# opencb/hpg-variant

Measured on AMD Instinct MI355X. Metric: variants/s chi2 assoc, higher is better.
Workload: dtype u8

## Files before the change

### hpg-variant_amd/csrc/hpgv_capi.hip

```cpp
#include "hpgv_internal.h"
#include <cstdlib>

extern "C" {

const char *hpgv_version(void) { return "hpgv-mi355x 0.1 (gfx950)"; }

int hpgv_device_count(void) {
    int n = 0;
    if (hipGetDeviceCount(&n) != hipSuccess) return -1;
    return n;
}

const char *hpgv_last_error(const hpgv_ctx *ctx) { return ctx ? ctx->err.c_str() : g_create_error.c_str(); }

static void read_environment(hpgv_ctx *ctx) {
    auto num = [](const char *name, long lo, long hi, long *out) { const char *e = getenv(name); if (e && *e) { long v = atol(e); *out = v < lo ? lo : v > hi ? hi : v; } };
    num("HPGV_BATCH_COPY", 0, 1, &ctx->batch_copy);
    num("HPGV_BATCH_FUSED", 0, 1, &ctx->batch_fused);
    num("HPGV_STATS_ALL2", 0, 1, &ctx->stats_all2);
    num("HPGV_ASSOC_ROWS", 0, 1, &ctx->assoc_rows);
    num("HPGV_PINNED_NONCOHERENT", 0, 1, &ctx->pinned_noncoherent);
    num("HPGV_VMM_TRACE", 0, 1, &ctx->vmm_trace);
    num("HPGV_DECODE_TILES", 0, 1, &ctx->decode_tiles);
#ifdef HPGV_ABLATION
// ... 127 lines not shown
        if (s->stream) (void)hipStreamDestroy(s->stream);
        delete s;
    }
    for (int i = 0; i < 4; ++i) if (ctx->ev[i]) (void)hipEventDestroy(ctx->ev[i]);
    delete ctx;
}

#ifdef HPGV_ABLATION
#define HPGV_SHIPPED_ONLY(ok, what)
#else
#define HPGV_SHIPPED_ONLY(ok, what) if (!(ok)) return fail(ctx, HPGV_ERR_UNSUPPORTED, what ": that form is an ablation build's (-DHPGV_ABLATION, tools/build_ablation.py)");
#endif

int hpgv_set_option(hpgv_ctx *ctx, const char *key, long value) {
    if (is_group(ctx) && key && !strcmp(key, "group_self_exchange")) { ctx->group_self_exchange = value ? 1 : 0; return HPGV_OK; }
    if (is_group(ctx) && key && !strcmp(key, "group_fake_ranks")) {
        if (value < 0 || value > 65536) return fail(ctx, HPGV_ERR_INVALID, "group_fake_ranks must be 0 (ranks by distinct device) or the number of members that share rank 0");
        std::lock_guard<std::mutex> lk(ctx->mu);
        if (ctx->grp) return fail(ctx, HPGV_ERR_STATE, "group_fake_ranks must be set before the group's communicator exists (hpgv_group_comm_init, the first group call)");
        ctx->group_fake_ranks = value;
        return HPGV_OK;
    }
    GROUP_ALL(ctx, hpgv_set_option(m_, key, value))
    if (!ctx || !key) return HPGV_ERR_INVALID;
    if (!strcmp(key, "row_align")) {
        if (value < 16 || (value & (value - 1))) return fail(ctx, HPGV_ERR_INVALID, "row_align must be a power of two >= 16");
        if (ctx->assoc.set || ctx->tdt.set || ctx->stats.set)
            return fail(ctx, HPGV_ERR_STATE, "row_align must be set before the cohort");
        ctx->row_align = value;
    } else if (!strcmp(key, "row_pad")) {
        if (value < 0 || value % 16 || value > 65536) return fail(ctx, HPGV_ERR_INVALID, "row_pad must be a multiple of 16 in [0, 65536]");
        if (ctx->assoc.set || ctx->tdt.set || ctx->stats.set)
            return fail(ctx, HPGV_ERR_STATE, "row_pad must be set before the cohort");
        ctx->row_pad = value;
    } else if (!strcmp(key, "variants_per_wave")) {
        if (value < 1 || value > 1024) return fail(ctx, HPGV_ERR_INVALID, "variants_per_wave out of range");
        ctx->vpw = value;
    } else if (!strcmp(key, "nontemporal")) {
        HPGV_SHIPPED_ONLY(value != 0, "nontemporal = 0")
        ctx->nontemporal = value ? 1 : 0;
    } else if (!strcmp(key, "profile")) {
        ctx->profile = value ? 1 : 0;
    } else if (!strcmp(key, "scan_unroll")) {
        if (value != 4 && value != 8 && value != 10 && value != 12 && value != 16)
            return fail(ctx, HPGV_ERR_INVALID, "scan_unroll must be one of 4, 8, 10, 12, 16");
        HPGV_SHIPPED_ONLY(value == 4, "scan_unroll other than 4")
        ctx->scan_unroll = value;
    } else if (!strcmp(key, "pipeline")) {
        HPGV_SHIPPED_ONLY(value != 0, "pipeline = 0")
        ctx->pipeline = value ? 1 : 0;
    } else if (!strcmp(key, "fisher_cut_exp")) {
        if (value < 12 || value > 300) return fail(ctx, HPGV_ERR_INVALID, "fisher_cut_exp must be in [12, 300]");
        ctx->fisher_cut_exp = value;
    } else if (!strcmp(key, "epi_complete")) {
        ctx->epi_complete = value ? 1 : 0;
    } else if (!strcmp(key, "epi_triples_mfma")) {
        ctx->epi_triples_mfma = value ? 1 : 0;
    } else if (!strcmp(key, "epi_pairs_mfma")) {
        ctx->epi_pairs_mfma = value ? 1 : 0;
    } else if (!strcmp(key, "epi_wide")) {
        if (value < 0 || value > 2) return fail(ctx, HPGV_ERR_INVALID, "epi_wide must be 0 (the packed kernels' limits), 1 (the wide kernel where the shape needs it) or 2 (the wide kernel for every listed-combination launch)");
        ctx->epi_wide = value;
    } else if (!strcmp(key, "epi_triples_1pass")) {
        if (value < 0 || value > 2) return fail(ctx, HPGV_ERR_INVALID, "epi_triples_1pass must be 0 (two passes), 1 (the cells nine at a time) or 2 (one pass, one wave per SIMD)");
        HPGV_SHIPPED_ONLY(value != 2, "epi_triples_1pass = 2")
        ctx->epi_triples_1pass = value;
    } else if (!strcmp(key, "scan_lds")) {
        if (value < 0 || value > 160 * 1024) return fail(ctx, HPGV_ERR_INVALID, "scan_lds must be in [0, 163840]");
        ctx->scan_lds = value;
    } else if (!strcmp(key, "batch_copy")) {
        ctx->batch_copy = value ? 1 : 0;
    } else if (!strcmp(key, "inflate_wave")) {
        if (value < 0 || value > 4) return fail(ctx, HPGV_ERR_INVALID, "inflate_wave must be 0 (lane per block), 1 (by the number of blocks), 2 (wave per block), 4 (wave per block, several symbols per round) or 3 (lane per block, symbol tables in LDS)");
        HPGV_SHIPPED_ONLY(value == 1 || value == 4, "inflate_wave other than 1 / 4 (a wave per block, several symbols per round)")
        ctx->inflate_wave = value;
    } else if (!strcmp(key, "tokenizer_tiles")) {
        if (value < 0 || value > 2) return fail(ctx, HPGV_ERR_INVALID, "tokenizer_tiles must be 2 (one sweep), 1 (two sweeps) or 0 (line by line)");
        HPGV_SHIPPED_ONLY(value == 1, "tokenizer_tiles other than 1 (two sweeps)")
        ctx->tokenizer_tiles = value;
    } else if (!strcmp(key, "fisher_width")) {
        if (value != 64 && value != 32 && value != 16 && value != 8) return fail(ctx, HPGV_ERR_INVALID, "fisher_width must be 64, 32, 16 or 8");
        HPGV_SHIPPED_ONLY(value == 16, "fisher_width other than 16")
        ctx->fisher_width = value;
    } else if (!strcmp(key, "batch_fused")) {
        ctx->batch_fused = value ? 1 : 0;
    } else if (!strcmp(key, "pipe_waves")) {
        if (value != 4 && value != 6 && value != 8) return fail(ctx, HPGV_ERR_INVALID, "pipe_waves must be 4, 6 or 8");
        HPGV_SHIPPED_ONLY(value == 4, "pipe_waves other than 4")
        ctx->pipe_waves = value;
    } else if (!strcmp(key, "persistent")) {
        HPGV_SHIPPED_ONLY(value == 0, "persistent = 1")
        ctx->persistent = value ? 1 : 0;
    } else if (!strcmp(key, "part_aligned_loads")) {
        HPGV_SHIPPED_ONLY(value == 0, "part_aligned_loads = 1")
        ctx->part_aligned = value ? 1 : 0;
    } else if (!strcmp(key, "pca_apply_vector")) {
        HPGV_SHIPPED_ONLY(value == 0, "pca_apply_vector = 1")
        ctx->pca_apply_vector = value ? 1 : 0;
    } else if (!strcmp(key, "blocks_per_cu")) {
        if (value < 1 || value > 8) return fail(ctx, HPGV_ERR_INVALID, "blocks_per_cu must be in 1..8");
        ctx->blocks_per_cu = value;
    } else {
        return fail(ctx, HPGV_ERR_INVALID, "unknown option '%s'", key);
    }
    return HPGV_OK;
}


int hpgv_set_cohort(hpgv_ctx *ctx, const uint8_t *condition, int n_samples) {
    HPGV_ABI_TRY
    GROUP_ALL(ctx, hpgv_set_cohort(m_, condition, n_samples))
    if (!ctx) return HPGV_ERR_INVALID;
    if (!condition || n_samples < 0) return fail(ctx, HPGV_ERR_INVALID, "bad cohort arguments");
    DeviceGuard g(ctx->device);
    int nA = 0, nU = 0;
    for (int j = 0; j < n_samples; ++j) {
        if (condition[j] == HPGV_COND_AFFECTED) nA++;
        else if (condition[j] == HPGV_COND_UNAFFECTED) nU++;
    }
    size_t segA = round_up((size_t)nA, 16), segU = round_up((size_t)nU, 16);
    size_t pitch = round_up(segA + segU, (size_t)ctx->row_align) + (size_t)ctx->row_pad;
    if (pitch == 0) pitch = (size_t)ctx->row_align;
    if (!pitch_supported(pitch)) return fail(ctx, HPGV_ERR_UNSUPPORTED, "cohort of %d samples exceeds the row-length limit", n_samples);
    Layout &L = ctx->assoc;
    ctx->n_perms = ctx->perm_rows = 0;
    ctx->n_covar = 0;
    ctx->has_pheno = false; ctx->lin_y.clear(); ctx->lin_cov.clear();
    L.n_samples = n_samples;
    L.pitch = pitch;
    L.col_of_pos.assign(pitch, -1);
    size_t a = 0, u = segA;
    for (int j = 0; j < n_samples; ++j) {
        if (condition[j] == HPGV_COND_AFFECTED) L.col_of_pos[a++] = j;
        else if (condition[j] == HPGV_COND_UNAFFECTED) L.col_of_pos[u++] = j;
    }
    ctx->nA = nA; ctx->nU = nU; ctx->chunksA = (int)(segA / 16);
    {
        std::vector<uint8_t> cond(round_up((size_t)n_samples, 16) + 16, (uint8_t)HPGV_COND_OTHER);
        for (int j = 0; j < n_samples; ++j) cond[(size_t)j] = condition[j] == HPGV_COND_AFFECTED ? 1 : condition[j] == HPGV_COND_UNAFFECTED ? 0 : 2;
        HIPCHK(ctx, ctx->d_cond.reserve(cond.size()));
        HIPCHK(ctx, hipMemcpy(ctx->d_cond.p, cond.data(), cond.size(), hipMemcpyHostToDevice));
    }
    return upload_layout(ctx, L);
    HPGV_ABI_CATCH(ctx)
}

int hpgv_assoc_layout(const hpgv_ctx *ctx, int *n_affected, int *n_unaffected, size_t *pitch) {
    ctx = first_member(ctx);
    if (!ctx) return HPGV_ERR_INVALID;
    if (!ctx->assoc.set) return fail(ctx, HPGV_ERR_STATE, "hpgv_set_cohort has not been called");
    if (n_affected) *n_affected = ctx->nA;
    if (n_unaffected) *n_unaffected = ctx->nU;
    if (pitch) *pitch = ctx->assoc.pitch;
    return HPGV_OK;
}

int hpgv_set_logfact(hpgv_ctx *ctx, const double *table, size_t n) {
    GROUP_ALL(ctx, hpgv_set_logfact(m_, table, n))
    if (!ctx) return HPGV_ERR_INVALID;
    if (!table || n == 0) return fail(ctx, HPGV_ERR_INVALID, "empty log-factorial table");
    DeviceGuard g(ctx->device);
    ctx->n_lf = 0;
    if (ctx->cap_lf < n) {
        if (ctx->d_lf_base) { (void)hipFree(ctx->d_lf_base); ctx->d_lf_base = nullptr; ctx->d_lf = nullptr; ctx->cap_lf = 0; }
        HIPCHK(ctx, hipMalloc(&ctx->d_lf_base, (n + 4) * sizeof(double)));
        HIPCHK(ctx, hipMemset(ctx->d_lf_base, 0, (n + 4) * sizeof(double)));
// ... 423 lines not shown
```

### hpg-variant_amd/csrc/hpgv_internal.h

```cpp
#pragma once
#include "../../include/hpgv.h"
#include "hpgv_kernels.h"
#include "hpgv_tdt_stats_kernels.h"
#include "hpgv_epi_kernels.h"

#include <hip/hip_runtime.h>
#include <cctype>

#include <algorithm>
#include <atomic>
#include <cmath>
#include <cstdarg>
#include <cstdio>
#include <cstring>
#include <mutex>
#include <new>
#include <string>
#include <vector>

namespace { thread_local std::string g_create_error; }

struct DevBuf {
    void *p = nullptr;
    size_t cap = 0;
// ... 74 lines not shown

struct TextMeta {
    char *base;
    size_t max_lines;
    TextMeta(const DevBuf &meta, int max_lines_) : base(meta.as<char>()), max_lines((size_t)max_lines_) {}
    static size_t bytes(int max_lines) { return 16 + ((size_t)max_lines + 2) * sizeof(uint64_t) + (size_t)max_lines * 10 * sizeof(uint32_t) + 16; }
    int *n_lines() const { return (int *)base; }
    unsigned long long *line_off() const { return (unsigned long long *)(base + 16); }
    uint32_t *field_off() const { return (uint32_t *)(base + 16 + (max_lines + 2) * sizeof(uint64_t)); }
};

struct Staged {
    const uint8_t *d_raw = nullptr;
    size_t raw_pitch = 0;
    const uint8_t *d_laid = nullptr;
    int which = 0;
    const uint8_t *d_isx = nullptr;
    int n = 0;
    size_t out_stride = 0;
    bool text = false;
};

struct EpiState {
    bool have_data = false, have_folds = false;
    int V = 0, nA = 0, nU = 0, num_folds = 0, W = 0, V_alloc = 0, n_chunks = 0;
    bool wide_only = false;
    int fold_cap = 0;
    int rank_fold_cap = 0;
    uint8_t *d_data = nullptr;
    uint32_t *d_planes = nullptr;
    uint32_t rev_off = 0;
    hpgv_epi_rank_info rank_info{};
    uint32_t *d_marg = nullptr;
    bool complete = false;
    hpgv::EpiChunk *d_chunks = nullptr;
    uint32_t *d_chunk_cls = nullptr;
    hpgv::EpiFold *d_folds = nullptr;
    uint32_t *d_group_w0 = nullptr;
    std::vector<int32_t> group_size;
    DevBuf cand;
    unsigned *d_cand_count = nullptr;
    unsigned cand_cap = 0;
    double *d_thr = nullptr;
    DevBuf tile_base;
};

struct hpgv_ctx {
    std::vector<hpgv_ctx *> members;
    hpgv_ctx *parent = nullptr;
    struct GroupState *grp = nullptr;
    long group_self_exchange = 0;
    long group_fake_ranks = 0;
    std::atomic<unsigned> deal_next{0};
    std::atomic<int> in_flight{0};
    int device = 0;
    mutable std::string err;
    std::mutex mu;
    long row_align = 16;
    long row_pad = 0;
    long vpw = 2;
    long nontemporal = 1;
    long profile = 0;
    std::mutex alias_mu;
    std::vector<std::pair<const char *, const char *>> text_alias;
    struct TextTiles { const char *d_text, *d_base; const void *d_tiles; uint64_t n_tiles; };
    std::vector<TextTiles> text_tiles;
    struct TextHeld { const char *host_text; Slot *slot; const char *d_text; const unsigned long long *d_line_off; int n_lines; };
    std::vector<TextHeld> text_held;
    long part_aligned = 0;
    long pca_apply_vector = 0;
    long scan_unroll = 4;
    long persistent = 0;
    long blocks_per_cu = 8;
    long pipeline = 1;
    long pipe_waves = 4;
    long fisher_cut_exp = 22;
    long epi_complete = 1;
    long epi_pairs_mfma = 1;
    long epi_triples_mfma = 1;
    long epi_wide = 0;
    long epi_triples_1pass = 1;
    long scan_lds = 0;
    long fisher_width = 16;
    long inflate_wave = 1;
    long tokenizer_tiles = 1;
    long batch_copy = 0;
    long batch_fused = 1;
    long batch_lds_max = 65536;
    long stats_all2 = 1;
    long assoc_rows = 1;
    long pinned_noncoherent = 0;
    long vmm_trace = 0;
    long decode_tiles = 1;
#ifdef HPGV_ABLATION
    long stats_rows = 0, stats_bs = 0, stats_debug = 0;
    long fisher_lds = 0;
    long inflate_lds_pad = 0, inflate_wave_wgs = 0, inflate_lane_wgs = 0;
#endif
    int n_cus = 256;
    Layout assoc;
    int nA = 0, nU = 0, chunksA = 0;
    DevBuf d_cond;
    DevBuf d_perm;
    int n_perms = 0, perm_rows = 0;
    DevBuf d_cov;
    int n_covar = 0;
    std::vector<double> lin_y, lin_cov;
    bool has_pheno = false;
    DevBuf d_lin;
    Layout tdt;
    hpgv::TdtPlan tdt_plan;
    DevBuf d_flips;
    int n_flips = 0, flip_rows = 0, flip_pitch = 0;
    int tdt_families = 0;
    DevBuf d_flip_tail;
    Layout stats;
    Layout sgroups;
    std::vector<uint32_t> sg_off;
    std::vector<int> sg_size;
    DevBuf d_sg_chunks;
    DevBuf d_group_of_col;
    bool all_grouped = false;
    Layout mendel;
    int mendel_trios = 0, mendel_pchunks = 0;
    hpgv::MendelLuts mendel_luts{};
    uint8_t *d_mendel_male = nullptr;
    double *d_lf = nullptr;
    double *d_lf_base = nullptr;
    size_t n_lf = 0;
    size_t cap_lf = 0;
    DevBuf d_thr;
    hipEvent_t ev[4] = {nullptr, nullptr, nullptr, nullptr};
    bool have_scan_ev = false, have_stats_ev = false;
    std::vector<Slot *> slots;
    uint32_t *d_sink = nullptr;
    uint32_t *d_crc_tab = nullptr;
    struct TokScratch {
        hipStream_t stream = nullptr;
        DevBuf blocks, line_off, extra;
    };
    std::mutex tok_mu;
    std::vector<TokScratch *> tok_scratch;
    struct GrowRange { char *base = nullptr; size_t reserved = 0, committed = 0; std::vector<hipMemGenericAllocationHandle_t> pieces; std::vector<size_t> sizes; };
    std::vector<GrowRange> grow;
    double filt_min_maf = -1.0, filt_max_missing = -1.0;
    long filt_max_mendel = -1;
    double filt_min_dom = -1.0, filt_min_rec = -1.0;
    std::mutex epi_mu;
    EpiState epi;
};

namespace {

[[maybe_unused]] int fail(const hpgv_ctx *ctx, int code, const char *fmt, ...) {
    char buf[512];
    va_list ap;
    va_start(ap, fmt);
    vsnprintf(buf, sizeof buf, fmt, ap);
    va_end(ap);
    if (ctx) {
        ctx->err = buf;
        if (ctx->parent) {
            std::lock_guard<std::mutex> lk(ctx->parent->mu);
            ctx->parent->err = buf;
        }
    } else g_create_error = buf;
// ... 193 lines not shown
```

### hpg-variant_amd/csrc/hpgv_scan_capi.hip

```cpp
#include "hpgv_internal.h"
#include <type_traits>
#include "hpgv_inherit_kernels.h"

namespace {

unsigned scan_blocks(const hpgv_ctx *ctx, int n_variants) {
    const long waves = ((long)n_variants + ctx->vpw - 1) / ctx->vpw;
    return (unsigned)((waves + 3) / 4);
}

const char *const kAligned16 = "device buffers must be 16-byte aligned";
int scan_checks(hpgv_ctx *ctx, int n_variants, const void *d_gt, const void *d_out, uintptr_t out_mask, const char *align_text, bool *go) {
    *go = false;
    if (n_variants < 0 || (n_variants > 0 && (!d_gt || !d_out))) return fail(ctx, HPGV_ERR_INVALID, "bad scan arguments");
    if (n_variants == 0) return HPGV_OK;
    if (((uintptr_t)d_gt & 15) || ((uintptr_t)d_out & out_mask)) return fail(ctx, HPGV_ERR_INVALID, "%s", align_text);
    *go = true;
    return HPGV_OK;
}

template <typename F>
void launch_nt(const hpgv_ctx *ctx, F &&f) {
    if (ctx->nontemporal) f(std::true_type{}); else f(std::false_type{});
}

}

extern "C" {


static Layout *pick_layout(hpgv_ctx *ctx, int which) {
    switch (which) {
        case HPGV_LAYOUT_ASSOC: return &ctx->assoc;
        case HPGV_LAYOUT_TDT: return &ctx->tdt;
        case HPGV_LAYOUT_STATS: return &ctx->stats;
        case HPGV_LAYOUT_STATS_GROUPS: return &ctx->sgroups;
        case HPGV_LAYOUT_MENDEL: return &ctx->mendel;
        case HPGV_LAYOUT_EPI: return &ctx->assoc;
        default: return nullptr;
    }
}

static void recode_of(const hpgv_ctx *ctx, int which, int *mode, int *p16) {
    *mode = hpgv::RECODE_NONE; *p16 = 0;
    if (which == HPGV_LAYOUT_TDT) { *mode = hpgv::RECODE_TDT; *p16 = ctx->tdt_plan.p16; }
    else if (which == HPGV_LAYOUT_STATS || which == HPGV_LAYOUT_STATS_GROUPS) { *mode = hpgv::RECODE_STATS; }
    else if (which == HPGV_LAYOUT_MENDEL) { *mode = hpgv::RECODE_MENDEL; }
    else if (which == HPGV_LAYOUT_EPI) { *mode = hpgv::RECODE_EPI; }
}

int hpgv_layout_dev(hpgv_ctx *ctx, int which, const uint8_t *d_src, size_t src_pitch, int n_variants,
                    uint8_t *d_dst, void *stream) {
    ctx = first_member(ctx);
    if (!ctx) return HPGV_ERR_INVALID;
    Layout *L = pick_layout(ctx, which);
    if (!L) return fail(ctx, HPGV_ERR_INVALID, "unknown layout %d", which);
    if (!L->set) return fail(ctx, HPGV_ERR_STATE, "layout %d has no cohort yet", which);
    if (n_variants < 0 || (n_variants > 0 && (!d_src || !d_dst))) return fail(ctx, HPGV_ERR_INVALID, "bad layout arguments");
    if (src_pitch < (size_t)L->n_samples) return fail(ctx, HPGV_ERR_INVALID, "src_pitch %zu < n_samples %d", src_pitch, L->n_samples);
    if (n_variants == 0) return HPGV_OK;
    DeviceGuard g(ctx->device);
    const int strict = (which == HPGV_LAYOUT_STATS || which == HPGV_LAYOUT_STATS_GROUPS) ? 0 : 1;
    int mode, p16;
    recode_of(ctx, which, &mode, &p16);
    const long slab = std::max(1L, (1L << 31) / (L->chunks > 0 ? L->chunks : 1));
    for (long off = 0; off < n_variants; off += slab) {
        const int n = (int)std::min(slab, (long)n_variants - off);
        const long total = (long)n * L->chunks;
        hipLaunchKernelGGL(hpgv::k_layout, dim3((unsigned)((total + 255) / 256)), dim3(256), 0, (hipStream_t)stream,
                           d_src + (size_t)off * src_pitch, src_pitch, n, L->pitch, L->chunks, L->d_col_of_pos(), strict, mode, p16,
                           d_dst + (size_t)off * L->pitch);
    }
    HIPCHK(ctx, hipGetLastError());
    return HPGV_OK;
}

static int synth_common(hpgv_ctx *ctx, uint64_t v0, int n_variants, size_t pitch, int chunks,
                        const int32_t *d_col, int mode, int p16, uint8_t *d_dst, hipStream_t st) {
    const long by_threads = (1L << 31) / (chunks > 0 ? chunks : 1);
    const int slab = (int)std::max(1L, std::min((long)(1 << 20), by_threads));
    HIPCHK(ctx, ctx->d_thr.reserve((size_t)(n_variants < slab ? n_variants : slab) * 3 * sizeof(uint32_t)));
    uint32_t *d_thr = ctx->d_thr.as<uint32_t>();
    for (int off = 0; off < n_variants; off += slab) {
        const int n = (n_variants - off) < slab ? (n_variants - off) : slab;
        hipLaunchKernelGGL(hpgv::k_synth_thresholds, dim3((n + 255) / 256), dim3(256), 0, st,
// ... 62 lines not shown
    unsigned blocks = scan_blocks(ctx, n_variants);
    if (ctx->persistent) {
        const unsigned cap = (unsigned)(ctx->n_cus * ctx->blocks_per_cu);
        const unsigned need = (unsigned)(((long)n_variants + 3) / 4);
        blocks = need < cap ? need : cap;
    }
    hipStream_t st = (hipStream_t)stream;
    const uint8_t *gt = d_gt;
    int4 *out = (int4 *)d_counts;
    const int cA = ctx->chunksA, ch = L.chunks;
    const size_t pitch = L.pitch;
#define HPGV_LAUNCH_PIPE(NT, U, W)                                                                \
    hipLaunchKernelGGL((hpgv::k_assoc_scan_pipe<NT, U, W>), dim3(blocks), dim3(256), 0, st, gt, pitch, \
                       n_variants, cA, ch, d_is_x, out, vpw)
#ifndef HPGV_ABLATION
    return launch_profiled(ctx, st, 0, [&] { HPGV_LAUNCH_PIPE(true, 4, 4); });
#else
#define HPGV_LAUNCH_ASSOC(NT, U, S)                                                              \
    hipLaunchKernelGGL((hpgv::k_assoc_scan<NT, U, S>), dim3(blocks), dim3(256), 0, st, gt, pitch, \
                       n_variants, cA, ch, d_is_x, out, vpw)
#define HPGV_DISPATCH_U(NT, S)                                                                   \
    switch (ctx->scan_unroll) {                                                                  \
        case 4: HPGV_LAUNCH_ASSOC(NT, 4, S); break;                                              \
        case 10: HPGV_LAUNCH_ASSOC(NT, 10, S); break;                                            \
        case 12: HPGV_LAUNCH_ASSOC(NT, 12, S); break;                                            \
        case 16: HPGV_LAUNCH_ASSOC(NT, 16, S); break;                                            \
        default: HPGV_LAUNCH_ASSOC(NT, 8, S); break;                                             \
    }
#define HPGV_PIPE_W(NT, U)                                                                       \
    do {                                                                                         \
        if (ctx->pipe_waves == 8) { HPGV_LAUNCH_PIPE(NT, U, 8); }                                \
        else if (ctx->pipe_waves == 6) { HPGV_LAUNCH_PIPE(NT, U, 6); }                           \
        else { HPGV_LAUNCH_PIPE(NT, U, 4); }                                                     \
    } while (0)
    if (ctx->pipeline && !ctx->persistent)
        return launch_profiled(ctx, st, 0, [&] {
            if (ctx->nontemporal) {
                if (ctx->scan_unroll <= 4) HPGV_PIPE_W(true, 4); else HPGV_PIPE_W(true, 5);
            } else {
                if (ctx->scan_unroll <= 4) HPGV_PIPE_W(false, 4); else HPGV_PIPE_W(false, 5);
            }
        });
    return launch_profiled(ctx, st, 0, [&] {
        if (ctx->nontemporal) {
            if (ctx->persistent) { HPGV_DISPATCH_U(true, true) } else { HPGV_DISPATCH_U(true, false) }
        } else {
            if (ctx->persistent) { HPGV_DISPATCH_U(false, true) } else { HPGV_DISPATCH_U(false, false) }
        }
    });
#undef HPGV_DISPATCH_U
#undef HPGV_PIPE_W
#undef HPGV_LAUNCH_ASSOC
#endif
#undef HPGV_LAUNCH_PIPE
}

int hpgv_assoc_chisq_dev(hpgv_ctx *ctx, const int32_t *d_counts, int n_variants, double *d_odds,
                         double *d_chisq, double *d_p, void *stream) {
    ctx = first_member(ctx);
    if (!ctx) return HPGV_ERR_INVALID;
    if (n_variants < 0 || (n_variants > 0 && (!d_counts || !d_odds || !d_chisq || !d_p)))
        return fail(ctx, HPGV_ERR_INVALID, "bad chisq arguments");
    if (n_variants == 0) return HPGV_OK;
    DeviceGuard g(ctx->device);
    hipStream_t st = (hipStream_t)stream;
    return launch_profiled(ctx, st, 1, [&] {
        hipLaunchKernelGGL(hpgv::k_assoc_chisq, dim3((n_variants + 255) / 256), dim3(256), 0, st,
                           (const int4 *)d_counts, n_variants, d_odds, d_chisq, d_p);
    });
}

int hpgv_assoc_fisher_dev(hpgv_ctx *ctx, const int32_t *d_counts, int n_variants, double *d_odds,
                          double *d_p, void *stream) {
    ctx = first_member(ctx);
    if (!ctx) return HPGV_ERR_INVALID;
    if (n_variants < 0 || (n_variants > 0 && (!d_counts || !d_odds || !d_p)))
        return fail(ctx, HPGV_ERR_INVALID, "bad fisher arguments");
    if (const int rc = logfact_check(ctx)) return rc;
    if (n_variants == 0) return HPGV_OK;
    DeviceGuard g(ctx->device);
    hipStream_t st = (hipStream_t)stream;
    const double cut = pow(10.0, -(double)ctx->fisher_cut_exp);
    return launch_profiled(ctx, st, 1, [&] {
        const long per_block = 4 * (64 / ctx->fisher_width);
        const unsigned blocks = (unsigned)(((long)n_variants + per_block - 1) / per_block);
#ifdef HPGV_ABLATION
        const unsigned pad = (unsigned)ctx->fisher_lds;
        if (ctx->fisher_width == 64)
            hipLaunchKernelGGL(hpgv::k_assoc_fisher<64>, dim3(blocks), dim3(256), pad, st, (const int4 *)d_counts, n_variants, ctx->d_lf, d_odds, d_p, cut);
        else if (ctx->fisher_width == 8)
            hipLaunchKernelGGL(hpgv::k_assoc_fisher<8>, dim3(blocks), dim3(256), pad, st, (const int4 *)d_counts, n_variants, ctx->d_lf, d_odds, d_p, cut);
        else if (ctx->fisher_width == 32)
            hipLaunchKernelGGL(hpgv::k_assoc_fisher<32>, dim3(blocks), dim3(256), pad, st, (const int4 *)d_counts, n_variants, ctx->d_lf, d_odds, d_p, cut);
        else
#else
        const unsigned pad = 0u;
#endif
            hipLaunchKernelGGL(hpgv::k_assoc_fisher<16>, dim3(blocks), dim3(256), pad, st, (const int4 *)d_counts, n_variants, ctx->d_lf, d_odds, d_p, cut);
    });
}


int hpgv_tdt_scan_dev(hpgv_ctx *ctx, const uint8_t *d_gt, int n_variants, const uint8_t *d_is_x,
                      int32_t *d_tu, void *stream) {
    ctx = first_member(ctx);
    if (!ctx) return HPGV_ERR_INVALID;
    if (!ctx->tdt.set) return fail(ctx, HPGV_ERR_STATE, "hpgv_set_families has not been called");
    bool go;
    if (const int rc = scan_checks(ctx, n_variants, d_gt, d_tu, 7, "device buffers must be aligned", &go); rc || !go) return rc;
    DeviceGuard g(ctx->device);
    hipStream_t st = (hipStream_t)stream;
    return launch_profiled(ctx, st, 0, [&] {
        ctx->tdt_plan.launch_scan(d_gt, ctx->tdt.pitch, n_variants, d_is_x, (int2 *)d_tu,
                                  (int)ctx->vpw, ctx->nontemporal != 0, st);
    });
}

int hpgv_tdt_stats_dev(hpgv_ctx *ctx, const int32_t *d_tu, int n_variants, double *d_odds,
                       double *d_chisq, double *d_p, void *stream) {
    ctx = first_member(ctx);
    if (!ctx) return HPGV_ERR_INVALID;
    if (n_variants < 0 || (n_variants > 0 && (!d_tu || !d_odds || !d_chisq || !d_p)))
        return fail(ctx, HPGV_ERR_INVALID, "bad tdt stats arguments");
    if (n_variants == 0) return HPGV_OK;
    DeviceGuard g(ctx->device);
    hipStream_t st = (hipStream_t)stream;
    return launch_profiled(ctx, st, 1, [&] {
        hipLaunchKernelGGL(hpgv::k_tdt_stats, dim3((n_variants + 255) / 256), dim3(256), 0, st,
                           (const int2 *)d_tu, n_variants, d_odds, d_chisq, d_p);
    });
}


static int stats_scan(hpgv_ctx *ctx, const Layout &L, const uint8_t *d_gt, int n_variants, uint32_t off, int chunks, size_t lds,
                      int32_t *d_counts8, hipStream_t st) {
    bool go;
    if (const int rc = scan_checks(ctx, n_variants, d_gt, d_counts8, 15, kAligned16, &go); rc || !go) return rc;
    DeviceGuard g(ctx->device);
    const int vpw = (int)ctx->vpw;
    const unsigned blocks = scan_blocks(ctx, n_variants);
    return launch_profiled(ctx, st, 0, [&] {
        launch_nt(ctx, [&](auto NT) {
            constexpr bool nt = decltype(NT)::value;
            if (ctx->pipeline)
                hipLaunchKernelGGL((hpgv::k_stats_scan_hs<nt>), dim3(blocks), dim3(256), nt ? lds : 0, st, d_gt, L.pitch, n_variants, off, chunks, (int4 *)d_counts8, vpw);
            else
                hipLaunchKernelGGL((hpgv::k_stats_scan<nt, kScanUnroll>), dim3(blocks), dim3(256), 0, st, d_gt, L.pitch, n_variants, off, chunks, (int4 *)d_counts8, vpw);
        });
    });
}

int hpgv_stats_scan_dev(hpgv_ctx *ctx, const uint8_t *d_gt, int n_variants, int32_t *d_counts8, void *stream) {
    ctx = first_member(ctx);
    if (!ctx) return HPGV_ERR_INVALID;
    if (!ctx->stats.set) return fail(ctx, HPGV_ERR_STATE, "hpgv_set_stats_cohort has not been called");
    const Layout &L = ctx->stats;
    const size_t scan_lds = ctx->scan_lds > 0 ? (size_t)ctx->scan_lds : (L.pitch >= 6656 ? (size_t)49152 : (size_t)0);
    return stats_scan(ctx, L, d_gt, n_variants, 0u, L.chunks, scan_lds, d_counts8, (hipStream_t)stream);
}

int hpgv_stats_scan_group_dev(hpgv_ctx *ctx, const uint8_t *d_gt, int n_variants, int group, int32_t *d_counts8, void *stream) {
    ctx = first_member(ctx);
    if (!ctx) return HPGV_ERR_INVALID;
    if (!ctx->sgroups.set) return fail(ctx, HPGV_ERR_STATE, "hpgv_set_stats_groups has not been called");
    if (group < 0 || (size_t)group >= ctx->sg_off.size()) return fail(ctx, HPGV_ERR_INVALID, "group %d out of range", group);
    const int chunks = (int)(round_up((size_t)ctx->sg_size[(size_t)group], 16) / 16);
    return stats_scan(ctx, ctx->sgroups, d_gt, n_variants, ctx->sg_off[(size_t)group], chunks, 0, d_counts8, (hipStream_t)stream);
}

int hpgv_stats_hwe_dev(hpgv_ctx *ctx, const int32_t *d_counts8, int n_variants, double *d_chi2,
                       double *d_p, void *stream) {
    ctx = first_member(ctx);
    if (!ctx) return HPGV_ERR_INVALID;
    if (n_variants < 0 || (n_variants > 0 && (!d_counts8 || !d_chi2 || !d_p)))
        return fail(ctx, HPGV_ERR_INVALID, "bad hwe arguments");
    if (n_variants == 0) return HPGV_OK;
    DeviceGuard g(ctx->device);
    hipStream_t st = (hipStream_t)stream;
    return launch_profiled(ctx, st, 1, [&] {
        hipLaunchKernelGGL(hpgv::k_stats_hwe, dim3((n_variants + 255) / 256), dim3(256), 0, st,
                           (const int4 *)d_counts8, n_variants, d_chi2, d_p);
// ... 152 lines not shown
```

Measured before the change: 136.7 million.

## Add packed Fisher kernel that load-balances tail sums across tables in a wave

Adds a new Fisher exact test kernel in which each wave handles four contingency tables. It locates the significant tail ranges with ballot-based window searches, then spreads the tail-term evaluation evenly across all 64 lanes through an LDS work list. It also uses a leaner exp with a cutoff derived from the tail-decay estimate. The aim is to cut lane imbalance when tables differ in tail length, at the cost of more LDS use and a more complex kernel. It becomes the default Fisher path, but chi-square association does not go through it.

```diff
diff --git a/hpg-variant_amd/csrc/hpgv_capi.hip b/hpg-variant_amd/csrc/hpgv_capi.hip
--- a/hpg-variant_amd/csrc/hpgv_capi.hip
+++ b/hpg-variant_amd/csrc/hpgv_capi.hip
@@ -233,6 +233,9 @@
         if (value != 64 && value != 32 && value != 16 && value != 8) return fail(ctx, HPGV_ERR_INVALID, "fisher_width must be 64, 32, 16 or 8");
         HPGV_SHIPPED_ONLY(value == 16, "fisher_width other than 16")
         ctx->fisher_width = value;
+    } else if (!strcmp(key, "fisher_packed")) {
+        HPGV_SHIPPED_ONLY(value != 0, "fisher_packed = 0")
+        ctx->fisher_packed = value ? 1 : 0;
     } else if (!strcmp(key, "batch_fused")) {
         ctx->batch_fused = value ? 1 : 0;
     } else if (!strcmp(key, "pipe_waves")) {
diff --git a/hpg-variant_amd/csrc/hpgv_fisher_kernels.h b/hpg-variant_amd/csrc/hpgv_fisher_kernels.h
--- /dev/null
+++ b/hpg-variant_amd/csrc/hpgv_fisher_kernels.h
@@ -0,0 +1,250 @@
+#pragma once
+#include "hpgv_kernels.h"
+
+namespace hpgv {
+
+constexpr int FISHER_PACK_TABLES = 4;
+constexpr int FISHER_PACK_TAILS = 2 * FISHER_PACK_TABLES;
+constexpr int FISHER_PACK_SLOTS = 64;
+
+struct alignas(16) FisherTail {
+    double konst; int pb8, n ;
+    int r1c, c1c, d0c, pq ;
+    int s16 , q , pad0, pad1;
+};
+
+__device__ __forceinline__ void fisher_wave_sync() {
+    __builtin_amdgcn_fence(__ATOMIC_RELEASE, "wavefront");
+    __builtin_amdgcn_wave_barrier();
+    __builtin_amdgcn_fence(__ATOMIC_ACQUIRE, "wavefront");
+}
+
+__device__ __forceinline__ double fisher_exp_lean(double e, const double *tab , bool keep) {
+    const double t = e * 0x1.71547652b82fep+6 + 0x1.8p+52;
+    const double kf = t - 0x1.8p+52;
+    const int ki = (int)(uint32_t)(uint64_t)__double_as_longlong(t);
+    double r = __builtin_fma(-kf, 0x1.62e42fe000000p-7, e);
+    r = __builtin_fma(-kf, 0x1.f473de6af278fp-36, r);
+    const double tj = tab[ki & 63];
+    double q = __builtin_fma(r, 1.0 / 120.0, 1.0 / 24.0);
+    q = __builtin_fma(r, q, 1.0 / 6.0);
+    q = __builtin_fma(r, q, 0.5);
+    q = __builtin_fma(r * r, q, r);
+    const double y = __builtin_fma(tj, q, tj);
+    return __builtin_ldexp(y, keep ? ki >> 6 : -4000);
+}
+
+
+__device__ __forceinline__ double fisher_get(double v, int lane, int k) { return __shfl(v, (lane & ~15) + k); }
+
+__device__ __forceinline__ void fisher_count2x16(bool p_lo, bool p_hi, int lane, int *left, int *right) {
+    const uint64_t bl = __ballot(p_lo), bh = __ballot(p_hi);
+    const uint32_t l = (((lane & 32) ? (uint32_t)(bl >> 32) : (uint32_t)bl) >> (lane & 16)) & 0xffffu;
+    const uint32_t h = (((lane & 32) ? (uint32_t)(bh >> 32) : (uint32_t)bh) >> (lane & 16)) & 0xffffu;
+    *left = __builtin_popcount(l & 0xffu) + __builtin_popcount(h & 0xffu);
+    *right = __builtin_popcount(l >> 8) + __builtin_popcount(h >> 8);
+}
+
+__device__ __forceinline__ bool fisher_windows_shared(const FisherTab &T, double thr , int mode, int obs, int lane,
+                                                      int *L1, int *R1, int *L2, int *R2) {
+    constexpr int W = 16;
+    const int sl = sub_lane<W>(lane), right = sl >> 3, j = sl & 7;
+    const int g1 = obs <= mode ? obs + 1 : 2 * mode - obs + 1, g2 = obs <= mode ? 2 * mode - obs : obs;
+    int w1 = g1 - W / 2, w2 = g2 - W / 2;
+    w1 = w1 > *R1 - W ? *R1 - W : w1; w1 = w1 < *L1 ? *L1 : w1;
+    w2 = w2 > *R2 - W ? *R2 - W : w2; w2 = w2 < *L2 ? *L2 : w2;
+    const int x = (right ? w2 : w1) + 2 * j, R = right ? *R2 : *R1;
+    const bool in_lo = x < R, in_hi = x + 1 < R;
+    double e_lo = 0.0, e_hi = 0.0;
+    if (in_lo) T.e2(x, &e_lo, &e_hi);
+    int c1, c2;
+    fisher_count2x16(in_lo && (right ? e_lo > thr : e_lo <= thr), in_hi && (right ? e_hi > thr : e_hi <= thr), lane, &c1, &c2);
+    int n1 = *R1 - w1, n2 = *R2 - w2;
+    n1 = n1 < 0 ? 0 : (n1 > W ? W : n1); n2 = n2 < 0 ? 0 : (n2 > W ? W : n2);
+    bool ok = true;
+    if (c1 == 0 && w1 > *L1) { *R1 = w1; ok = false; }
+    else if (c1 == n1 && w1 + n1 < *R1) { *L1 = w1 + n1; ok = false; }
+    else { *L1 = w1 + c1; *R1 = w1 + c1; }
+    if (c2 == 0 && w2 > *L2) { *R2 = w2; ok = false; }
+    else if (c2 == n2 && w2 + n2 < *R2) { *L2 = w2 + n2; ok = false; }
+    else { *L2 = w2 + c2; *R2 = w2 + c2; }
+    return ok;
+}
+
+__device__ __forceinline__ int fisher_probe_pos(int w, int s, int k) { return w + (k >> 1) * s + (k & 1); }
+__device__ __forceinline__ void fisher_tail_ends(const FisherTab &T, double thr1, double thr2, int L1, int R1, int g1, int s1,
+                                                 int L2, int R2, int g2, int s2, int lane, int *end1, int *end2) {
+    constexpr int W = 16;
+    const int sl = sub_lane<W>(lane), right = sl >> 3, j = sl & 7;
+    const double thr = right ? thr2 : thr1;
+    int w1 = g1 - 4 * s1, w2 = g2 - 4 * s2;
+    while (R1 > L1 || R2 > L2) {
+        w1 = w1 > R1 - 2 - 7 * s1 ? R1 - 2 - 7 * s1 : w1; w1 = w1 < L1 ? L1 : w1;
+        w2 = w2 > R2 - 2 - 7 * s2 ? R2 - 2 - 7 * s2 : w2; w2 = w2 < L2 ? L2 : w2;
+        const int x = right ? w2 + j * s2 : w1 + j * s1, R = right ? R2 : R1;
+        const bool in_lo = x < R, in_hi = x + 1 < R;
+        double e_lo = 0.0, e_hi = 0.0;
+        if (in_lo) T.e2(x, &e_lo, &e_hi);
+        int c1, c2;
+        fisher_count2x16(in_lo && (right ? e_lo > thr : e_lo <= thr), in_hi && (right ? e_hi > thr : e_hi <= thr), lane, &c1, &c2);
+        const int p1 = fisher_probe_pos(w1, s1, c1), p2 = fisher_probe_pos(w2, s2, c2);
+        const int nL1 = c1 > 0 ? fisher_probe_pos(w1, s1, c1 - 1) + 1 : L1, nR1 = (c1 < W && p1 < R1) ? p1 : R1;
+        const int nL2 = c2 > 0 ? fisher_probe_pos(w2, s2, c2 - 1) + 1 : L2, nR2 = (c2 < W && p2 < R2) ? p2 : R2;
+        L1 = nL1; R1 = nR1; L2 = nL2; R2 = nR2;
+        s1 = (R1 - L1 + 7) >> 3; s1 = s1 < 2 ? 2 : s1; w1 = L1;
+        s2 = (R2 - L2 + 7) >> 3; s2 = s2 < 2 ? 2 : s2; w2 = L2;
+    }
+    *end1 = L1; *end2 = L2;
+}
+
+template <bool RAGGED>
+__device__ __forceinline__ void fisher_quad(int i, const int (&P)[FISHER_PACK_TAILS + 1], const FisherTail *D, double *S,
+                                            const double *__restrict__ lf, const double *exp_tab) {
+    int t = 0;
+#pragma unroll
+    for (int j = 1; j < FISHER_PACK_TAILS; ++j) t += i >= P[j] ? 1 : 0;
+    const FisherTail f = D[t];
+    const int m = i - f.pq;
+    const int r = m & (FISHER_PACK_SLOTS - 1), blk = m - r;
+    const int left = f.q - blk, h = left < FISHER_PACK_SLOTS ? left : FISHER_PACK_SLOTS;
+    const int pA = 2 * blk + r, pB = pA + h;
+    const int remA = f.n - 2 * pA, remB = f.n - 2 * pB;
+    const uint32_t a0 = (uint32_t)(f.pb8 + pA * f.s16), a1 = (uint32_t)f.r1c - a0, a2 = (uint32_t)f.c1c - a0, a3 = (uint32_t)f.d0c + a0;
+    const uint32_t sB = (uint32_t)((RAGGED && remB < 1 ? 0 : h) * f.s16);
+    const char *b = reinterpret_cast<const char *>(lf) - 16;
+    double2 q0, q1, q2, q3, u0, u1, u2, u3;
+    __builtin_memcpy(&q0, b + a0, 16); __builtin_memcpy(&q1, b + a1, 16); __builtin_memcpy(&q2, b + a2, 16); __builtin_memcpy(&q3, b + a3, 16);
+    __builtin_memcpy(&u0, b + (a0 + sB), 16); __builtin_memcpy(&u1, b + (a1 - sB), 16); __builtin_memcpy(&u2, b + (a2 - sB), 16); __builtin_memcpy(&u3, b + (a3 + sB), 16);
+    const double e0lo = f.konst - q0.x - q1.y - q2.y - q3.x, e0hi = f.konst - q0.y - q1.x - q2.x - q3.y;
+    const double e1lo = f.konst - u0.x - u1.y - u2.y - u3.x, e1hi = f.konst - u0.y - u1.x - u2.x - u3.y;
+    const int jlo = f.s16 < 0 ? 1 : 0, jhi = 1 - jlo;
+    const double s0 = fisher_exp_lean(e0lo, exp_tab, !RAGGED || remA > jlo) + fisher_exp_lean(e0hi, exp_tab, !RAGGED || remA > jhi);
+    const double s1 = fisher_exp_lean(e1lo, exp_tab, !RAGGED || remB > jlo) + fisher_exp_lean(e1hi, exp_tab, !RAGGED || remB > jhi);
+    S[t * FISHER_PACK_SLOTS + r] += s0 + s1;
+}
+
+__global__ __launch_bounds__(256) void k_assoc_fisher_packed(const int4 *__restrict__ counts, int n,
+                                                             const double *__restrict__ lf,
+                                                             double *__restrict__ odds,
+                                                             double *__restrict__ pval, double ln_cut ) {
+    constexpr int W = 16;
+    __shared__ double exp_tab[64];
+    __shared__ double sums[4][FISHER_PACK_TAILS * FISHER_PACK_SLOTS];
+    __shared__ FisherTail tails[4][FISHER_PACK_TAILS];
+    const int lane = threadIdx.x & 63, wv = threadIdx.x >> 6, sl = sub_lane<W>(lane), sv = lane / W;
+    double *S = sums[wv];
+    FisherTail *D = tails[wv];
+    if (threadIdx.x < 64) exp_tab[threadIdx.x] = k_exp2_j64[threadIdx.x];
+#pragma unroll
+    for (int j = 0; j < FISHER_PACK_TAILS; ++j) S[j * FISHER_PACK_SLOTS + lane] = 0.0;
+    __syncthreads();
+    const long wave = (long)blockIdx.x * 4 + wv;
+    const long v = wave * FISHER_PACK_TABLES + sv;
+    const bool live = v < n;
+    int4 c4 = make_int4(0, 0, 0, 0);
+    if (live) c4 = counts[v];
+    const int a = c4.x, b = c4.y, c = c4.z, d = c4.w;
+
+    const int r1 = a + b, r2 = c + d, c1 = a + c, nn = r1 + r2;
+    const int lo = (c1 - r2) > 0 ? (c1 - r2) : 0;
+    const int hi = r1 < c1 ? r1 : c1;
+    FisherTab T;
+    T.lf = lf; T.xt = exp_tab; T.r1 = r1; T.c1 = c1; T.d0 = r2 - c1;
+    const int idx0 = sl == 0 ? r1 : sl == 1 ? r2 : sl == 2 ? c1 : sl == 3 ? nn - c1
+                   : sl == 4 ? a : sl == 5 ? r1 - a : sl == 6 ? c1 - a : sl == 7 ? T.d0 + a : nn;
+    const double tv0 = lf[idx0];
+    T.konst = fisher_get(tv0, lane, 0) + fisher_get(tv0, lane, 1) + fisher_get(tv0, lane, 2) + fisher_get(tv0, lane, 3) - fisher_get(tv0, lane, 8);
+    const double thr = T.konst - fisher_get(tv0, lane, 4) - fisher_get(tv0, lane, 5) - fisher_get(tv0, lane, 6) - fisher_get(tv0, lane, 7) + 9.9999995000000333e-08;
+    double whole = 0.0;
+    int xL = lo, xR = hi + 1, nL = 0, nR = 0;
+    const bool is_short = hi - lo < 8 * W;
+    if (is_short) {
+        double part = 0.0;
+        for (int x = lo + sl; x <= hi; x += W) {
+            const double ex = T.e(x);
+            if (ex <= thr) part += fisher_exp(ex, exp_tab);
+        }
+        whole = sub_sum_f64<W>(part);
+    } else {
+        const double prod = (double)(r1 + 1) * (double)(c1 + 1), den = (double)(nn + 2);
+        double md = __builtin_floor(prod / den);
+        const double rem = __builtin_fma(-md, den, prod);
+        md += rem >= den ? 1.0 : (rem < 0.0 ? -1.0 : 0.0);
+        int mode = (int)md;
+        mode = mode < lo ? lo : (mode > hi ? hi : mode);
+        int L1 = lo, R1 = mode + 1, L2 = mode + 1, R2 = hi + 1;
+        if (fisher_windows_shared(T, thr, mode, a, lane, &L1, &R1, &L2, &R2)) { xL = L1; xR = L2; }
+        else fisher_boundaries<W>(T, thr, L1, R1, L2, R2, lane, &xL, &xR);
+        const bool hasL = xL > lo, hasR = xR <= hi;
+        const int xf = (sl & 4) ? (hasR ? xR : hi) : (hasL ? xL - 1 : lo), kf = sl & 3;
+        const double tv1 = lf[kf == 0 ? xf : kf == 1 ? r1 - xf : kf == 2 ? c1 - xf : T.d0 + xf];
+        const double eL = T.konst - fisher_get(tv1, lane, 0) - fisher_get(tv1, lane, 1) - fisher_get(tv1, lane, 2) - fisher_get(tv1, lane, 3);
+        const double eR = T.konst - fisher_get(tv1, lane, 4) - fisher_get(tv1, lane, 5) - fisher_get(tv1, lane, 6) - fisher_get(tv1, lane, 7);
+        const float fn = (float)nn;
+        const float var2 = 2.0f * ((float)r1 * (float)r2 * __builtin_amdgcn_rcpf(fn)) * ((float)c1 * (float)(nn - c1) * __builtin_amdgcn_rcpf(fn)) * __builtin_amdgcn_rcpf(fn - 1.0f);
+        const float spread = -(float)ln_cut * var2;
+        const float dL0 = (float)(mode - (xL - 1)), dR0 = (float)(xR - mode);
+        const int dL = (int)__builtin_fminf(__builtin_amdgcn_sqrtf(dL0 * dL0 + spread), 1.0e6f);
+        const int dR = (int)__builtin_fminf(__builtin_amdgcn_sqrtf(dR0 * dR0 + spread), 1.0e6f);
+        int endL, endR;
+        fisher_tail_ends(T, eL + ln_cut, eR + ln_cut, lo, hasL ? xL - 1 : lo, mode - dL, (dL >> 5) + 2,
+                         hasR ? xR + 1 : hi + 1, hi + 1, mode + dR, (dR >> 5) + 2, lane, &endL, &endR);
+        nL = hasL ? xL - endL : 0;
+        nR = hasR ? endR - xR : 0;
+        nL = (nL + 3) & ~3; nL = nL > xL - lo ? xL - lo : nL;
+        nR = (nR + 3) & ~3; nR = nR > hi + 1 - xR ? hi + 1 - xR : nR;
+    }
+
+    const int qL = (nL + 3) >> 2, qR = (nR + 3) >> 2;
+    int P[FISHER_PACK_TAILS + 1];
+    P[0] = 0;
+#pragma unroll
+    for (int k = 0; k < FISHER_PACK_TABLES; ++k) {
+        P[2 * k + 1] = P[2 * k] + __builtin_amdgcn_readlane(qL, k * W);
+        P[2 * k + 2] = P[2 * k + 1] + __builtin_amdgcn_readlane(qR, k * W);
+    }
+    const int total = P[FISHER_PACK_TAILS];
+    if (sl < 2) {
+        const int t = 2 * sv + sl;
+        int pq = 0;
+#pragma unroll
+        for (int j = 1; j < FISHER_PACK_TAILS; ++j) pq = t == j ? P[j] : pq;
+        FisherTail f;
+        f.konst = T.konst; f.pb8 = (sl ? xR + 2 : xL) << 3; f.n = sl ? nR : nL;
+        f.r1c = (T.r1 + 3) << 3; f.c1c = (T.c1 + 3) << 3; f.d0c = T.d0 << 3; f.pq = pq;
+        f.s16 = sl ? 16 : -16; f.q = sl ? qR : qL; f.pad0 = 0; f.pad1 = 0;
+        D[t] = f;
+    }
+    const bool ragged = __ballot(((nL | nR) & 3) != 0) != 0ull;
+    fisher_wave_sync();
+
+    const int iters = (total + 63) >> 6;
+    if (!ragged) {
+        for (int it = 0; it < iters; ++it) {
+            const int i = it * 64 + lane;
+            if (i < total) fisher_quad<false>(i, P, D, S, lf, exp_tab);
+            fisher_wave_sync();
+        }
+    } else {
+        for (int it = 0; it < iters; ++it) {
+            const int i = it * 64 + lane;
+            if (i < total) fisher_quad<true>(i, P, D, S, lf, exp_tab);
+            fisher_wave_sync();
+        }
+    }
+
+    double acc = 0.0;
+    {
+        const int t = lane >> 3, j = lane & 7;
+#pragma unroll
+        for (int k = 0; k < FISHER_PACK_SLOTS / 8; ++k) acc += S[t * FISHER_PACK_SLOTS + j + 8 * k];
+    }
+    const double tailsum = sub_sum_f64<W>(acc);
+    const double sum = is_short ? whole : tailsum;
+    if (live && sl == 0) {
+        odds[v] = assoc_odds(a, b, c, d);
+        pval[v] = sum > 1.0 ? 1.0 : sum;
+    }
+}
+
+}
diff --git a/hpg-variant_amd/csrc/hpgv_internal.h b/hpg-variant_amd/csrc/hpgv_internal.h
--- a/hpg-variant_amd/csrc/hpgv_internal.h
+++ b/hpg-variant_amd/csrc/hpgv_internal.h
@@ -180,6 +180,7 @@
     long epi_triples_1pass = 1;
     long scan_lds = 0;
     long fisher_width = 16;
+    long fisher_packed = 1;
     long inflate_wave = 1;
     long tokenizer_tiles = 1;
     long batch_copy = 0;
diff --git a/hpg-variant_amd/csrc/hpgv_scan_capi.hip b/hpg-variant_amd/csrc/hpgv_scan_capi.hip
--- a/hpg-variant_amd/csrc/hpgv_scan_capi.hip
+++ b/hpg-variant_amd/csrc/hpgv_scan_capi.hip
@@ -1,6 +1,7 @@
 #include "hpgv_internal.h"
 #include <type_traits>
 #include "hpgv_inherit_kernels.h"
+#include "hpgv_fisher_kernels.h"
 
 namespace {
 
@@ -229,21 +230,30 @@
     hipStream_t st = (hipStream_t)stream;
     const double cut = pow(10.0, -(double)ctx->fisher_cut_exp);
     return launch_profiled(ctx, st, 1, [&] {
-        const long per_block = 4 * (64 / ctx->fisher_width);
-        const unsigned blocks = (unsigned)(((long)n_variants + per_block - 1) / per_block);
 #ifdef HPGV_ABLATION
+        if (!ctx->fisher_packed || ctx->fisher_width != 16) {
+            const long per_block = 4 * (64 / ctx->fisher_width);
+            const unsigned blocks = (unsigned)(((long)n_variants + per_block - 1) / per_block);
+            const unsigned pad = (unsigned)ctx->fisher_lds;
+            if (ctx->fisher_width == 64)
+                hipLaunchKernelGGL(hpgv::k_assoc_fisher<64>, dim3(blocks), dim3(256), pad, st, (const int4 *)d_counts, n_variants, ctx->d_lf, d_odds, d_p, cut);
+            else if (ctx->fisher_width == 8)
+                hipLaunchKernelGGL(hpgv::k_assoc_fisher<8>, dim3(blocks), dim3(256), pad, st, (const int4 *)d_counts, n_variants, ctx->d_lf, d_odds, d_p, cut);
+            else if (ctx->fisher_width == 32)
+                hipLaunchKernelGGL(hpgv::k_assoc_fisher<32>, dim3(blocks), dim3(256), pad, st, (const int4 *)d_counts, n_variants, ctx->d_lf, d_odds, d_p, cut);
+            else
+                hipLaunchKernelGGL(hpgv::k_assoc_fisher<16>, dim3(blocks), dim3(256), pad, st, (const int4 *)d_counts, n_variants, ctx->d_lf, d_odds, d_p, cut);
+            return;
+        }
         const unsigned pad = (unsigned)ctx->fisher_lds;
-        if (ctx->fisher_width == 64)
-            hipLaunchKernelGGL(hpgv::k_assoc_fisher<64>, dim3(blocks), dim3(256), pad, st, (const int4 *)d_counts, n_variants, ctx->d_lf, d_odds, d_p, cut);
-        else if (ctx->fisher_width == 8)
-            hipLaunchKernelGGL(hpgv::k_assoc_fisher<8>, dim3(blocks), dim3(256), pad, st, (const int4 *)d_counts, n_variants, ctx->d_lf, d_odds, d_p, cut);
-        else if (ctx->fisher_width == 32)
-            hipLaunchKernelGGL(hpgv::k_assoc_fisher<32>, dim3(blocks), dim3(256), pad, st, (const int4 *)d_counts, n_variants, ctx->d_lf, d_odds, d_p, cut);
-        else
 #else
         const unsigned pad = 0u;
 #endif
-            hipLaunchKernelGGL(hpgv::k_assoc_fisher<16>, dim3(blocks), dim3(256), pad, st, (const int4 *)d_counts, n_variants, ctx->d_lf, d_odds, d_p, cut);
+        const long per_block = 4 * hpgv::FISHER_PACK_TABLES;
+        const unsigned blocks = (unsigned)(((long)n_variants + per_block - 1) / per_block);
+        const double ln_cut = -(double)ctx->fisher_cut_exp * 2.302585092994045684;
+        (void)cut;
+        hipLaunchKernelGGL(hpgv::k_assoc_fisher_packed, dim3(blocks), dim3(256), pad, st, (const int4 *)d_counts, n_variants, ctx->d_lf, d_odds, d_p, ln_cut);
     });
 }
 
```

New measurement: 136.9 million, median of 2. About the same (+0.1%).
